# daxiongpro/EPNet

Hardware: AMD Instinct MI355X
Metric: SA-stack points/sec per GPU (16384-pt KITTI scene) + % HBM roofline (higher is better)
Workload: dtype f32

## Files before the change

### epnet_amd/_lib.py

```python
import ctypes
import os

_HERE = os.path.dirname(os.path.abspath(__file__))
LIB_PATH = os.environ.get("EPNET_HIP_LIB") or os.path.join(_HERE, "lib", "libepnet_hip.so")

_vp = ctypes.c_void_p
_i = ctypes.c_int
_f = ctypes.c_float
_sz = ctypes.c_size_t
_i64 = ctypes.c_int64

SIGNATURES = {
    "epnet_abi_version": (_i, []),
    "epnet_strerror": (ctypes.c_char_p, [_i]),
    "epnet_last_hip_error": (ctypes.c_char_p, []),
    "epnet_furthest_point_sampling": (_i, [_i, _i, _i, _vp, _vp, _vp, _vp]),
    "epnet_gather_points": (_i, [_i, _i, _i, _i, _vp, _vp, _vp, _vp]),
    "epnet_gather_points_grad": (_i, [_i, _i, _i, _i, _vp, _vp, _vp, _vp]),
    "epnet_ball_query": (_i, [_i, _i, _i, _f, _i, _vp, _vp, _vp, _vp]),
    "epnet_ball_query_workspace_bytes": (_sz, [_i, _i, _i]),
    "epnet_ball_query_ws": (_i, [_i, _i, _i, _f, _i, _vp, _vp, _vp, _vp, _sz, _vp]),
    "epnet_group_points": (_i, [_i, _i, _i, _i, _i, _vp, _vp, _vp, _vp]),
    "epnet_group_points_grad": (_i, [_i, _i, _i, _i, _i, _vp, _vp, _vp, _vp]),
    "epnet_group_concat": (_i, [_i, _i, _i, _i, _i, _vp, _vp, _vp, _vp, _vp, _i, _vp]),
# ... 5 lines not shown
    "epnet_group_concat_grad_ws": (_i, [_i, _i, _i, _i, _i, _vp, _vp, _vp, _i, _vp, _sz, _vp]),
    "epnet_three_nn": (_i, [_i, _i, _i, _vp, _vp, _vp, _vp, _vp]),
    "epnet_three_nn_workspace_bytes": (_sz, [_i, _i, _i]),
    "epnet_three_nn_ws": (_i, [_i, _i, _i, _vp, _vp, _vp, _vp, _vp, _sz, _vp]),
    "epnet_three_interpolate": (_i, [_i, _i, _i, _i, _vp, _vp, _vp, _vp, _vp]),
    "epnet_three_interpolate_grad": (_i, [_i, _i, _i, _i, _vp, _vp, _vp, _vp, _vp]),
    "epnet_three_interpolate_grad_workspace_bytes": (_sz, [_i, _i, _i]),
    "epnet_three_interpolate_grad_ws": (_i, [_i, _i, _i, _i, _vp, _vp, _vp, _vp, _vp, _sz, _vp]),
    "epnet_group_linear": (_i, [_i, _i, _i, _i, _i, _vp, _vp, _vp, _vp, _vp, _vp, _vp, _vp]),
    "epnet_group_linear_grad_w": (_i, [_i, _i, _i, _i, _i, _vp, _vp, _vp, _vp, _vp, _vp]),
    "epnet_feature_gather": (_i, [_i, _i, _i, _i, _i, _i, _i, _vp, _vp, _vp, _vp, _vp, _vp]),
    "epnet_feature_gather_grad": (_i, [_i, _i, _i, _i, _i, _i, _vp, _vp, _vp, _vp]),
    "epnet_pool_max": (_i, [ctypes.c_longlong, _i, _vp, _vp, _vp, _vp]),
    "epnet_pool_max_grad": (_i, [ctypes.c_longlong, _i, _vp, _vp, _vp, _vp]),
    "epnet_scene_index_bytes": (_sz, [_i, _i]),
    "epnet_scene_index_build": (_i, [_i, _i, _vp, _vp, _sz, _vp]),
    "epnet_scene_index_build_gathered": (_i, [_i, _i, _i, _vp, _vp, _vp, _vp, _sz, _vp]),
    "epnet_furthest_point_sampling_indexed": (_i, [_i, _i, _i, _vp, _vp, _sz, _vp, _vp, _vp]),
    "epnet_sample_centres": (_i, [_i, _i, _i, _vp, _vp, _sz, _vp, _vp, _vp, _vp]),
    "epnet_sample_centres_chain": (_i, [_i, _i, _i, _vp, _vp, _sz, _vp, _vp, _vp, _vp, _vp, _i, _vp]),
    "epnet_group_concat_multi": (_i, [_i, _i, _i, _i, _i, _vp, _vp, _vp, _vp, _vp, _vp, _i, _vp]),
    "epnet_ball_query_indexed_multi": (_i, [_i, _i, _i, _i, _vp, _vp, _vp, _vp, _vp, _sz, _vp, _vp]),
    "epnet_ball_query_ordered": (_i, [_i, _i, _i, _i, _vp, _vp, _vp, _vp, _vp, _sz, _vp, _sz, _vp, _vp]),
    "epnet_three_nn_indexed": (_i, [_i, _i, _i, _vp, _vp, _vp, _sz, _vp, _sz, _vp, _vp, _vp]),
    "epnet_ball_query_indexed": (_i, [_i, _i, _i, _f, _i, _vp, _vp, _vp, _sz, _vp, _vp]),
    "epnet_boxes_overlap_bev": (_i, [_i, _vp, _i, _vp, _vp, _vp]),
    "epnet_boxes_iou_bev": (_i, [_i, _vp, _i, _vp, _vp, _vp]),
    "epnet_boxes_iou3d": (_i, [_i, _vp, _i, _vp, _vp, _vp]),
    "epnet_boxes_iou3d_pairs": (_i, [_i, _vp, _vp, _vp, _vp]),
    "epnet_aug_roi_by_noise": (_i, [_i, _i, _f, _vp, _vp, _vp, _vp, _vp, _vp, _vp, _vp]),
    "epnet_rpn_proposals_workspace_bytes": (_sz, [_i, _i, _i, _i]),
    "epnet_rpn_proposals": (_i, [_i, _i, _vp, _vp, _vp, _i, _i, _i, _f, _i, _vp, _sz, _vp, _vp, _vp, _vp]),
    "epnet_nms_workspace_bytes": (_sz, [_i]),
    "epnet_nms": (_i, [_vp, _i, _f, _vp, _sz, _vp, _vp, _vp]),
    "epnet_nms_normal": (_i, [_vp, _i, _f, _vp, _sz, _vp, _vp, _vp]),
    "epnet_roipool3d_workspace_bytes": (_sz, [_i, _i, _i]),
    "epnet_roipool3d": (_i, [_i, _i, _i, _i, _i, _vp, _vp, _vp, _vp, _vp, _vp, _sz, _vp]),
    "epnet_pts_in_boxes3d_host": (_i, [_vp, _vp, _vp, _i64, _i64]),
    "epnet_roipool3d_host": (_i, [_vp, _vp, _vp, _vp, _vp, _vp, _i64, _i64, _i64, _i64]),
}

_lib = None


class EpnetError(RuntimeError):
    pass
# ... 30 lines not shown
```

### epnet_amd/csrc/ball_query.hip

```cpp
#include <stdlib.h>

#include "common.h"
#include "dpp.h"
#include "spatial.h"

namespace epnet {

constexpr int kBqTile = 2048;
constexpr int kBqThreads = 256;

template <int CPW>
__global__ __launch_bounds__(kBqThreads) void ball_query_kernel(int n, int m, float radius2, int nsample,
                                                                const float *__restrict__ new_xyz,
                                                                const float *__restrict__ xyz,
                                                                int *__restrict__ idx) {
    __shared__ float tile[kBqTile * 3];
    const int lane = threadIdx.x & 63, wave = threadIdx.x >> 6;
    const int bs = blockIdx.y;
    xyz += (size_t)bs * n * 3;
    new_xyz += (size_t)bs * m * 3;
    idx += (size_t)bs * m * nsample;

    const int c0 = (blockIdx.x * (kBqThreads / 64) + wave) * CPW;
    float cx[CPW], cy[CPW], cz[CPW];
// ... 325 lines not shown
        for (int q0 = 0; q0 < nq; q0 += 64) {
            const int qd = q0 + lane;
            const bool qnear = qd < nq && box_near(qboxes + qd * 6, cx, cy, cz, r2);
            const unsigned long long qmask = __ballot(qnear);
            if (!qmask) continue;
            const int nqc = (int)__popcll(qmask);
            if (qnear) quads[popc_below(qmask)] = qd;
            __builtin_amdgcn_wave_barrier();
            for (int s0 = 0; s0 < nqc; s0 += 16) {
                const int slot = s0 + (lane >> 2);
                int bid = 0;
                bool bnear = false;
                if (slot < nqc) {
                    bid = quads[slot] * 4 + (lane & 3);
                    bnear = box_near(boxes + bid * 6, cx, cy, cz, r2);
                }
                scan_buckets(__ballot(bnear), [&](int l) { return __builtin_amdgcn_readlane(bid, l); });
            }
            __builtin_amdgcn_wave_barrier();
        }
    }
}

__device__ __forceinline__ void bq_emit_list(int lane, const int *hits, int cnt, int nsample, int *__restrict__ out) {
    __builtin_amdgcn_wave_barrier();
    const int mine = lane < cnt ? hits[lane] : 0x7fffffff;
    int rank = 0;
    for (int j = 0; j < cnt; ++j) rank += __builtin_amdgcn_readlane(mine, j) < mine ? 1 : 0;
    if (lane < cnt && rank < nsample) out[rank] = mine;
    int first = 0;
    if (cnt) first = __builtin_amdgcn_readlane(mine, (int)__builtin_ctzll(__ballot(lane < cnt && rank == 0)));
    for (int l = cnt + lane; l < nsample; l += 64) out[l] = first;
}

template <int RM>
__device__ __forceinline__ int bq_select_smallest(int lane, int *hits, int cnt, int nsample, int np) {
    __builtin_amdgcn_wave_barrier();
    int key[RM];
#pragma unroll
    for (int r = 0; r < RM; ++r) key[r] = (r * 64 < cnt && r * 64 + lane < cnt) ? hits[r * 64 + lane] : 0x7fffffff;
    int lo = 0, hi = np;
    while (hi - lo > 1) {
        const int mid = (lo + hi) >> 1;
        int c = 0;
#pragma unroll
        for (int r = 0; r < RM; ++r)
            if (r * 64 < cnt) c += (int)__popcll(__ballot(key[r] < mid));
        if (c >= nsample) hi = mid;
        else lo = mid;
    }
    __builtin_amdgcn_wave_barrier();
    int base = 0;
#pragma unroll
    for (int r = 0; r < RM; ++r)
        if (r * 64 < cnt) {
            const bool sel = key[r] < hi;
            const unsigned long long sm = __ballot(sel);
            if (sel) hits[base + popc_below(sm)] = key[r];
            base += (int)__popcll(sm);
        }
    return hi;
}

template <int DPL>
__device__ __forceinline__ void bq_bitmap_search(int lane, int np, float r2, int nsample, float cx, float cy, float cz,
                                                 const float4 *__restrict__ sorted, const float *__restrict__ boxes,
                                                 const float *__restrict__ qboxes, int *__restrict__ out, unsigned *bits,
                                                 int *quads) {
#pragma unroll
    for (int w = 0; w < DPL; ++w) bits[lane * DPL + w] = 0u;
    __builtin_amdgcn_wave_barrier();
    bq_walk<DPL>(lane, np, r2, cx, cy, cz, sorted, boxes, qboxes, quads, [&](const float4 &p, float d2) {
        if (d2 < r2) {
            const int k = __float_as_int(p.w);
            atomicOr(&bits[k >> 5], 1u << (k & 31));
        }
    });
    __builtin_amdgcn_wave_barrier();
    int bc = 0;
#pragma unroll 8
    for (int i = 0; i < DPL; ++i) bc += __popc(bits[lane * DPL + i]);
    const int incl = wave_inclusive_scan(bc);
    const int total = __builtin_amdgcn_readlane(incl, 63);
    int pos = incl - bc;
    int mine_first = 0x7fffffff;
    if (bc > 0 && (pos < nsample || pos == 0)) {
        for (int i = 0; i < DPL; ++i) {
            unsigned ww = bits[lane * DPL + i];
            if (ww && mine_first == 0x7fffffff) mine_first = (lane * DPL + i) * 32 + (int)__builtin_ctz(ww);
            while (ww && pos < nsample) {
                const int bit = (int)__builtin_ctz(ww);
                ww &= ww - 1u;
                out[pos++] = (lane * DPL + i) * 32 + bit;
            }
            if (pos >= nsample) break;
        }
    }
    const unsigned long long have = __ballot(bc > 0);
    int first = 0;
    if (have) first = __builtin_amdgcn_readlane(mine_first, (int)__builtin_ctzll(have));
    for (int l = total + lane; l < nsample; l += 64) out[l] = first;
}

template <int K>
struct BqScales {
    float r2[K];
    int nsample[K];
    int *idx[K];
};

template <int DPL, int K>
__global__ __launch_bounds__(kQThreads) void bq_query_kernel(int np, int m, BqScales<K> sc,
                                                             const float *__restrict__ new_xyz,
                                                             const float4 *__restrict__ sorted,
                                                             const float *__restrict__ boxes,
                                                             const float *__restrict__ qboxes,
                                                             const float4 *__restrict__ order, int npc) {
    __shared__ unsigned s_bits[kQThreads / 64][64 * DPL];
    __shared__ int s_quads[kQThreads / 64][64];
    __shared__ int s_hits[kQThreads / 64][K][64];
    const int lane = threadIdx.x & 63, wave = threadIdx.x >> 6;
    int wg_x, bs;
    xcd_scene_map(wg_x, bs);
    int ci = wg_x * (kQThreads / 64) + wave;
    if (ci >= m) return;
    sorted += (size_t)bs * np;
    boxes += (size_t)bs * (np / 64) * 6;
    qboxes += (size_t)bs * (np / 256) * 6;
    float cx, cy, cz;
    if (order) {
        const float4 e = order[(size_t)bs * npc + ci];
        ci = __float_as_int(e.w);
        cx = e.x; cy = e.y; cz = e.z;
    } else {
        const float *c = new_xyz + ((size_t)bs * m + ci) * 3;
        cx = c[0]; cy = c[1]; cz = c[2];
    }
    float r2max = sc.r2[0];
#pragma unroll
    for (int k = 1; k < K; ++k) r2max = fmaxf(r2max, sc.r2[k]);
    int cnt[K];
#pragma unroll
    for (int k = 0; k < K; ++k) cnt[k] = 0;
    bq_walk<DPL>(lane, np, r2max, cx, cy, cz, sorted, boxes, qboxes, s_quads[wave], [&](const float4 &p, float d2) {
        if (!__ballot(d2 < r2max)) return;
#pragma unroll
        for (int k = 0; k < K; ++k) {
            const bool hit = d2 < sc.r2[k];
            const unsigned long long hm = __ballot(hit);
            if (hm) {
                const int pos = cnt[k] + popc_below(hm);
                if (hit && pos < 64) s_hits[wave][k][pos] = __float_as_int(p.w);
                cnt[k] += (int)__popcll(hm);
            }
        }
    });
#pragma unroll
    for (int k = 0; k < K; ++k) {
        int *out = sc.idx[k] + ((size_t)bs * m + ci) * sc.nsample[k];
        if (cnt[k] <= 64)
            bq_emit_list(lane, s_hits[wave][k], cnt[k], sc.nsample[k], out);
        else
            bq_bitmap_search<DPL>(lane, np, sc.r2[k], sc.nsample[k], cx, cy, cz, sorted, boxes, qboxes, out, s_bits[wave],
                                  s_quads[wave]);
    }
}

template <int DPL, int K, bool kStream>
__global__ __launch_bounds__(kQThreads) void bq_query2_kernel(int np, int m, BqScales<K> sc,
                                                              const float *__restrict__ new_xyz,
                                                              const float4 *__restrict__ sorted,
                                                              const float *__restrict__ boxes,
                                                              const float *__restrict__ qboxes,
                                                              const float4 *__restrict__ order, int npc) {
    constexpr int CAP = kStream ? (K == 1 ? 512 : 256) : 64, kStepAppends = 128;
    constexpr int kBitWords = kStream ? 0 : 64 * DPL;
    __shared__ unsigned s_pool[kQThreads / 64][kBitWords + 2 * K * CAP];
    __shared__ int s_quads[kQThreads / 64][2][64];
    const int lane = threadIdx.x & 63, wave = threadIdx.x >> 6;
    int wg_x, bs;
    xcd_scene_map(wg_x, bs);
    const int ci0 = (wg_x * (kQThreads / 64) + wave) * 2;
    if (ci0 >= m) return;
    const bool two = ci0 + 1 < m;
    sorted += (size_t)bs * np;
    boxes += (size_t)bs * (np / 64) * 6;
    qboxes += (size_t)bs * (np / 256) * 6;
    float ax, ay, az, bx_, by_, bz_;
    int out0 = ci0, out1 = ci0 + 1;
    if (order) {
        const float4 e0 = order[(size_t)bs * npc + ci0], e1 = order[(size_t)bs * npc + ci0 + (two ? 1 : 0)];
        ax = e0.x; ay = e0.y; az = e0.z;
        bx_ = e1.x; by_ = e1.y; bz_ = e1.z;
        out0 = __float_as_int(e0.w);
        out1 = __float_as_int(e1.w);
    } else {
        const float *c0 = new_xyz + ((size_t)bs * m + ci0) * 3;
        const float *c1 = two ? c0 + 3 : c0;
        ax = c0[0]; ay = c0[1]; az = c0[2];
        bx_ = c1[0]; by_ = c1[1]; bz_ = c1[2];
// ... 106 lines not shown
            }
            __builtin_amdgcn_wave_barrier();
        }
    }
#ifdef EPNET_BQ_STATS
    const unsigned long long st_1 = __builtin_amdgcn_s_memtime();
#endif
#pragma unroll
    for (int e = 0; e < 2; ++e) {
        if (e == 1 && !two) break;
        const float cx = e ? bx_ : ax, cy = e ? by_ : ay, cz = e ? bz_ : az;
#pragma unroll
        for (int k = 0; k < K; ++k) {
            int *out = sc.idx[k] + ((size_t)bs * m + (e ? out1 : out0)) * sc.nsample[k];
            int *hits = hits_of + (e * K + k) * CAP;
            if constexpr (kStream) {
                if (cnt[e][k] > 64) {
                    bq_select_smallest<CAP / 64>(lane, hits, cnt[e][k], sc.nsample[k], np);
                    cnt[e][k] = sc.nsample[k];
#ifdef EPNET_BQ_STATS
                    st_sel = true;
#endif
                }
                bq_emit_list(lane, hits, cnt[e][k], sc.nsample[k], out);
            } else {
                if (cnt[e][k] <= 64) {
                    bq_emit_list(lane, hits, cnt[e][k], sc.nsample[k], out);
                } else {
#ifdef EPNET_BQ_STATS
                    st_again = true;
#endif
                    bq_bitmap_search<DPL>(lane, np, sc.r2[k], sc.nsample[k], cx, cy, cz, sorted, boxes, qboxes, out, s_pool[wave],
                                          s_quads[wave][0]);
                }
            }
        }
    }
#ifdef EPNET_BQ_STATS
    {
        const unsigned long long st_3 = __builtin_amdgcn_s_memtime();
        if (lane == 0) {
            const int o = st_again ? 8 : (st_sel ? 4 : 0);
            atomicAdd(&g_bq_stats[o + 0], 1ull);
            atomicAdd(&g_bq_stats[o + 1], st_1 - st_0);
            atomicAdd(&g_bq_stats[o + 2], st_3 - st_1);
            atomicAdd(&g_bq_stats[o + 3], (unsigned long long)st_rows);
            atomicMax(&g_bq_stats[12], st_3 - st_0);
        }
    }
#endif
}

}

using namespace epnet;

extern "C" int epnet_ball_query(int b, int n, int m, float radius, int nsample, const float *new_xyz,
                                const float *xyz, int *idx, epnet_stream_t stream) {
    EPNET_REQUIRE(b >= 0 && n >= 0 && m >= 0 && nsample >= 0);
// ... 12 lines not shown
    }
    return check_launch("ball_query");
}


int epnet::spatial_index_launch(int b, int n, int np, const float *xyz, float4 *sorted, float *boxes, float *qboxes,
                                hipStream_t s, int n_src, const int *src_idx, float *gathered) {
    if (n <= 4096) {
        constexpr int T = 256, cells = 1 << 12;
        const size_t stage = (np & 255) == 0 ? (size_t)(np / 4 < 512 ? np / 4 : 512) * sizeof(float4) : 0;
        hipLaunchKernelGGL((bq_index_kernel<T, 12>), dim3(b), dim3(T), (size_t)(cells + cells / (cells / T) + 64) * sizeof(int) + stage, s,
                           n, np, xyz, sorted, boxes, qboxes, n_src, src_idx, gathered);
    } else {
        constexpr int T = 1024, cells = 1 << 14;
        const size_t stage = (n <= T * 16 && (np & 255) == 0) ? (size_t)(np / 4) * sizeof(float4) : 0;
        hipLaunchKernelGGL((bq_index_kernel<T, 14>), dim3(b), dim3(T), (size_t)(cells + cells / (cells / T) + 64) * sizeof(int) + stage, s,
                           n, np, xyz, sorted, boxes, qboxes, n_src, src_idx, gathered);
    }
    return check_launch("spatial index");
}

template <int K>
static int bq_query_launch(int b, int np, int m, const BqScales<K> &sc, const float *new_xyz, const float4 *sorted,
                           hipStream_t s, const float4 *order = nullptr, int npc = 0) {
    const float *boxes = (const float *)(sorted + (size_t)b * np);
    const float *qboxes = boxes + (size_t)b * (np / 64) * 6;
    const char *pair_str = getenv("EPNET_BQ_PAIR");
    const int pair_env = pair_str ? atoi(pair_str) : -1;
    const bool pair = pair_env >= 0 ? pair_env != 0 : (long long)b * m >= 65536;
    const char *pad_str = getenv("EPNET_BQ_PAD_KB");
    const size_t pad = pad_str ? (size_t)atoi(pad_str) * 1024 : 0;
    if (pair) {
        dim3 grid(div_up(div_up(m, 2), kQThreads / 64), b);
        bool stream = np > 16384;
        if (const char *e = getenv("EPNET_BQ_STREAM")) stream = atoi(e) != 0;
        for (int k = 0; k < K; ++k) stream = stream && sc.nsample[k] <= 64;
#define EPNET_BQ2(D_)                                                                                                                   \
    do {                                                                                                                                \
        if (stream)                                                                                                                     \
            hipLaunchKernelGGL((bq_query2_kernel<D_, K, true>), grid, dim3(kQThreads), pad, s, np, m, sc, new_xyz, sorted, boxes, qboxes, \
                               order, npc);                                                                                             \
        else                                                                                                                            \
            hipLaunchKernelGGL((bq_query2_kernel<D_, K, false>), grid, dim3(kQThreads), pad, s, np, m, sc, new_xyz, sorted, boxes,       \
                               qboxes, order, npc);                                                                                     \
    } while (0)
        switch (np / 2048) {
            case 1: EPNET_BQ2(1); break;
            case 2: EPNET_BQ2(2); break;
            case 4: EPNET_BQ2(4); break;
            case 8: EPNET_BQ2(8); break;
            case 16: EPNET_BQ2(16); break;
            default: EPNET_BQ2(32); break;
        }
#undef EPNET_BQ2
        return check_launch("ball_query query");
    }
    dim3 grid(div_up(m, kQThreads / 64), b);
#define EPNET_BQ(D_) hipLaunchKernelGGL((bq_query_kernel<D_, K>), grid, dim3(kQThreads), pad, s, np, m, sc, new_xyz, sorted, boxes, qboxes, order, npc)
    switch (np / 2048) {
        case 1: EPNET_BQ(1); break;
        case 2: EPNET_BQ(2); break;
        case 4: EPNET_BQ(4); break;
        case 8: EPNET_BQ(8); break;
        case 16: EPNET_BQ(16); break;
        default: EPNET_BQ(32); break;
    }
#undef EPNET_BQ
    return check_launch("ball_query query");
}

extern "C" size_t epnet_scene_index_bytes(int b, int n) { return scene_index_bytes(b, n); }

extern "C" int epnet_scene_index_build(int b, int n, const float *xyz, void *index, size_t index_bytes,
                                       epnet_stream_t stream) {
    const size_t need = scene_index_bytes(b, n);
    EPNET_REQUIRE(need != 0 && xyz && index);
    if (index_bytes < need) return EPNET_ENOMEM;
    if (((uintptr_t)index & 15) != 0) return EPNET_EINVAL;
    EPNET_REQUIRE(b <= 65535);
    const int np = scene_index_np(n);
    float4 *sorted = (float4 *)index;
// ... 35 lines not shown
extern "C" int epnet_ball_query_indexed_multi(int b, int n, int m, int nscales, const float *radii, const int *nsamples,
                                              const float *new_xyz, const float *xyz, const void *index,
                                              size_t index_bytes, int *const *idx, epnet_stream_t stream) {
    EPNET_REQUIRE(nscales >= 0 && (nscales == 0 || (radii && nsamples && idx)));
    const size_t need = scene_index_bytes(b, n);
    bool fused = nscales == 2 && need != 0 && index && m > 0 && nsamples[0] > 0 && nsamples[1] > 0;
    if (!fused) {
        for (int k = 0; k < nscales; ++k) {
            const int rc = epnet_ball_query_indexed(b, n, m, radii[k], nsamples[k], new_xyz, xyz, index, index_bytes, idx[k], stream);
            if (rc) return rc;
        }
        return EPNET_OK;
    }
    EPNET_REQUIRE(new_xyz && idx[0] && idx[1]);
    if (index_bytes < need) return EPNET_ENOMEM;
    EPNET_REQUIRE(b <= 65535);
    BqScales<2> sc;
    for (int k = 0; k < 2; ++k) {
        sc.r2[k] = radii[k] * radii[k];
        sc.nsample[k] = nsamples[k];
        sc.idx[k] = idx[k];
    }
    return bq_query_launch<2>(b, scene_index_np(n), m, sc, new_xyz, (const float4 *)index, (hipStream_t)stream);
}

extern "C" int epnet_ball_query_ordered(int b, int n, int m, int nscales, const float *radii, const int *nsamples,
                                        const float *new_xyz, const float *xyz, const void *index, size_t index_bytes,
                                        const void *centre_index, size_t centre_index_bytes, int *const *idx,
                                        epnet_stream_t stream) {
    EPNET_REQUIRE(nscales >= 0 && (nscales == 0 || (radii && nsamples && idx)));
    const size_t need = scene_index_bytes(b, n), need_c = scene_index_bytes(b, m);
    bool ordered = (nscales == 1 || nscales == 2) && need != 0 && need_c != 0 && index && centre_index && m > 0;
    for (int k = 0; ordered && k < nscales; ++k) ordered = nsamples[k] > 0 && idx[k] != nullptr;
    const char *force = getenv("EPNET_BQ_ORDERED");
    if (force ? atoi(force) == 0 : n <= 16384) ordered = false;
    if (!ordered) return epnet_ball_query_indexed_multi(b, n, m, nscales, radii, nsamples, new_xyz, xyz, index, index_bytes, idx, stream);
    if (index_bytes < need || centre_index_bytes < need_c) return EPNET_ENOMEM;
    EPNET_REQUIRE(b <= 65535);
    const int np = scene_index_np(n), npc = scene_index_np(m);
    if (nscales == 1) {
        BqScales<1> sc;
        sc.r2[0] = radii[0] * radii[0];
        sc.nsample[0] = nsamples[0];
        sc.idx[0] = idx[0];
        return bq_query_launch<1>(b, np, m, sc, new_xyz, (const float4 *)index, (hipStream_t)stream, (const float4 *)centre_index, npc);
    }
// ... 42 lines not shown
```

### epnet_amd/csrc/common.h

```cpp
#pragma once
#include <hip/hip_runtime.h>
#include <stdint.h>

#include "epnet_ops.h"

namespace epnet {

constexpr int kWave = 64;

int record_hip_error(hipError_t e, const char *where);

inline int check_launch(const char *where) {
    hipError_t e = hipGetLastError();
    if (e != hipSuccess) return record_hip_error(e, where);
    return EPNET_OK;
}

inline int div_up(int a, int b) { return (a + b - 1) / b; }
inline long long div_up64(long long a, long long b) { return (a + b - 1) / b; }

__device__ __forceinline__ int lane_id() { return threadIdx.x & (kWave - 1); }

__device__ __forceinline__ int popc_below(unsigned long long mask) {
    return __builtin_amdgcn_mbcnt_hi((unsigned)(mask >> 32), __builtin_amdgcn_mbcnt_lo((unsigned)mask, 0));
}

__device__ __forceinline__ void store_stream(float *dst, float x, float y, float z, float w) {
    typedef float f4 __attribute__((ext_vector_type(4)));
    const f4 v = {x, y, z, w};
    __builtin_nontemporal_store(v, reinterpret_cast<f4 *>(dst));
}

__device__ __forceinline__ void xcd_scene_map(int &wg_x, int &bs) {
// ... 42 lines not shown
```

### epnet_amd/csrc/group.hip

```cpp
#include <stdlib.h>

#include "common.h"
#include "spatial.h"
#include "runsum.h"

namespace epnet {

constexpr int kGThreads = 256;
constexpr int kGChan = 16;

__global__ __launch_bounds__(kGThreads) void gather_rows_vec4_kernel(int c, int n, int p, size_t ostride,
                                                                     const float *__restrict__ points,
                                                                     const int *__restrict__ idx,
                                                                     float *__restrict__ out) {
    int wg_x, wg_y, bs;
    xcd_scene_map3(wg_x, wg_y, bs);
    const int c0 = wg_y * kGChan;
    const int q4 = wg_x * kGThreads + threadIdx.x;
    if (q4 * 4 >= p) return;
    const int4 id = *reinterpret_cast<const int4 *>(idx + (size_t)bs * p + (size_t)q4 * 4);
    const int cend = min(c, c0 + kGChan);
    const float *src = points + ((size_t)bs * c + c0) * n;
    float *dst = out + (size_t)bs * ostride + (size_t)c0 * p + (size_t)q4 * 4;
#pragma unroll 4
// ... 568 lines not shown
    return launch_gather_rows(b, c, n, npoints, points, idx, out, (hipStream_t)stream, "gather_points");
}

extern "C" int epnet_gather_points_grad(int b, int c, int n, int npoints, const float *grad_out, const int *idx,
                                        float *grad_points, epnet_stream_t stream) {
    EPNET_REQUIRE(b >= 0 && c >= 0 && n >= 0 && npoints >= 0);
    return launch_scatter_rows(b, c, n, npoints, grad_out, idx, grad_points, (hipStream_t)stream, "gather_points_grad");
}

extern "C" int epnet_group_points(int b, int c, int n, int npoints, int nsample, const float *points, const int *idx,
                                  float *out, epnet_stream_t stream) {
    EPNET_REQUIRE(b >= 0 && c >= 0 && n >= 0 && npoints >= 0 && nsample >= 0);
    return launch_gather_rows(b, c, n, (long long)npoints * nsample, points, idx, out, (hipStream_t)stream,
                              "group_points");
}

extern "C" int epnet_group_points_grad(int b, int c, int n, int npoints, int nsample, const float *grad_out,
                                       const int *idx, float *grad_points, epnet_stream_t stream) {
    EPNET_REQUIRE(b >= 0 && c >= 0 && n >= 0 && npoints >= 0 && nsample >= 0);
    return launch_scatter_rows(b, c, n, (long long)npoints * nsample, grad_out, idx, grad_points, (hipStream_t)stream,
                               "group_points_grad");
}

static int launch_group_xyz(int b, int n, int npoints, int nsample, long long p, size_t ostride, const float *xyz,
                            const float *new_xyz, const int *idx, float *out, hipStream_t s) {
    if (nsample % 4 == 0 && (((uintptr_t)idx | (uintptr_t)out) % 16 == 0) && (ostride % 4 == 0))
        hipLaunchKernelGGL(group_xyz_centred_vec4_kernel, dim3((unsigned)div_up64(p / 4, kGThreads), b), dim3(kGThreads), 0, s, n,
                           npoints, nsample, ostride, xyz, new_xyz, idx, out);
    else
        hipLaunchKernelGGL(group_xyz_centred_kernel, dim3((unsigned)div_up64(p, kGThreads), b), dim3(kGThreads), 0, s, n, npoints,
                           nsample, ostride, xyz, new_xyz, idx, out);
    return check_launch("group_concat xyz");
}

extern "C" int epnet_group_concat(int b, int c, int n, int npoints, int nsample, const float *xyz, const float *new_xyz,
                                  const float *features, const int *idx, float *out, int use_xyz, epnet_stream_t stream) {
    EPNET_REQUIRE(b >= 0 && c >= 0 && n >= 0 && npoints >= 0 && nsample >= 0);
    EPNET_REQUIRE(use_xyz || c > 0);
    const long long p = (long long)npoints * nsample;
    if (b == 0 || p == 0) return EPNET_OK;
    EPNET_REQUIRE(idx && out && (c == 0 || features) && (!use_xyz || (xyz && new_xyz)));
    EPNET_REQUIRE(n > 0);
    if (p > 0x7fffffffll || b > 65535) return EPNET_ELIMIT;
    hipStream_t s = (hipStream_t)stream;
    const int ch0 = use_xyz ? 3 : 0;
    const size_t ostride = (size_t)(ch0 + c) * (size_t)p;
    if (use_xyz) {
// ... 184 lines not shown
```

### epnet_amd/pointnet2_cuda.py

```python
import torch

from . import _lib
from ._tensor import dev_ptr, need, on_device_of, writes

_F, _I = torch.float32, torch.int32


@writes("idx")
def ball_query_wrapper(b, n, m, radius, nsample, new_xyz, xyz, idx):
    pn, px, pi = dev_ptr(new_xyz, "new_xyz", _F), dev_ptr(xyz, "xyz", _F), dev_ptr(idx, "idx", _I)
    need(new_xyz, b * m * 3, "new_xyz"); need(xyz, b * n * 3, "xyz"); need(idx, b * m * nsample, "idx")
    l = _lib.lib()
    ws_bytes = l.epnet_ball_query_workspace_bytes(b, n, m)
    with on_device_of(xyz) as s:
        if ws_bytes:
            ws = torch.empty((ws_bytes,), dtype=torch.uint8, device=xyz.device)
            _lib.check(l.epnet_ball_query_ws(b, n, m, radius, nsample, pn, px, pi, ws.data_ptr(), ws_bytes, s), "ball_query")
        else:
            _lib.check(l.epnet_ball_query(b, n, m, radius, nsample, pn, px, pi, s), "ball_query")
    return 1


@writes("out")
def group_points_wrapper(b, c, n, npoints, nsample, points, idx, out):
# ... 182 lines not shown
                       "sample_centres")
    return 1


@writes("idxs")
def ball_query_multi_wrapper(b, n, m, radii, nsamples, new_xyz, xyz, index, idxs):
    import ctypes
    pn, pxyz = dev_ptr(new_xyz, "new_xyz", _F), dev_ptr(xyz, "xyz", _F)
    need(new_xyz, b * m * 3, "new_xyz"); need(xyz, b * n * 3, "xyz")
    k = len(radii)
    assert len(nsamples) == k and len(idxs) == k
    ptrs = []
    for ns, t in zip(nsamples, idxs):
        ptrs.append(dev_ptr(t, "idx", _I))
        need(t, b * m * ns, "idx")
    px, nb = _index_args(index, xyz)
    c_r = (ctypes.c_float * k)(*[float(r) for r in radii])
    c_n = (ctypes.c_int * k)(*[int(x) for x in nsamples])
    c_p = (ctypes.c_void_p * k)(*ptrs)
    with on_device_of(xyz) as s:
        _lib.check(_lib.lib().epnet_ball_query_indexed_multi(b, n, m, k, ctypes.cast(c_r, ctypes.c_void_p),
                                                             ctypes.cast(c_n, ctypes.c_void_p), pn, pxyz, px, nb,
                                                             ctypes.cast(c_p, ctypes.c_void_p), s), "ball_query")
    return 1


@writes("idxs")
def ball_query_ordered_wrapper(b, n, m, radii, nsamples, new_xyz, xyz, index, centre_index, idxs):
    import ctypes
    pn, pxyz = dev_ptr(new_xyz, "new_xyz", _F), dev_ptr(xyz, "xyz", _F)
    need(new_xyz, b * m * 3, "new_xyz"); need(xyz, b * n * 3, "xyz")
    k = len(radii)
    assert len(nsamples) == k and len(idxs) == k
    ptrs = []
    for ns, t in zip(nsamples, idxs):
        ptrs.append(dev_ptr(t, "idx", _I))
        need(t, b * m * ns, "idx")
    px, nb = _index_args(index, xyz)
    pc, nc = _index_args(centre_index, new_xyz)
    c_r = (ctypes.c_float * k)(*[float(r) for r in radii])
    c_n = (ctypes.c_int * k)(*[int(x) for x in nsamples])
    c_p = (ctypes.c_void_p * k)(*ptrs)
    with on_device_of(xyz) as s:
        _lib.check(_lib.lib().epnet_ball_query_ordered(b, n, m, k, ctypes.cast(c_r, ctypes.c_void_p), ctypes.cast(c_n, ctypes.c_void_p),
                                                     pn, pxyz, px, nb, pc, nc, ctypes.cast(c_p, ctypes.c_void_p), s), "ball_query")
    return 1
# ... 166 lines not shown
```

### epnet_amd/sa_stack.py

```python
import os

import torch

from . import pointnet2_cuda as ext

RPN_NPOINTS = (4096, 1024, 256, 64)
RPN_RADII = ((0.1, 0.5), (0.5, 1.0), (1.0, 2.0), (2.0, 4.0))
RPN_NSAMPLES = ((16, 32), (16, 32), (16, 32), (16, 32))
RPN_FEAT_CHANNELS = (0, 96, 256, 512)
RPN_FP = ((1024, 64, 256), (512, 256, 1024), (512, 1024, 4096), (256, 4096, 16384))


CONFIGS = {
    2: dict(n=16384, npoints=RPN_NPOINTS, radii=RPN_RADII, nsamples=RPN_NSAMPLES, feat_channels=RPN_FEAT_CHANNELS),
    5: dict(n=65536, npoints=(16384,), radii=((0.5,),), nsamples=((64,),), feat_channels=(64,)),
}


def sa_algorithmic_bytes(n=16384, npoints=RPN_NPOINTS, nsamples=RPN_NSAMPLES, feat_channels=RPN_FEAT_CHANNELS):
    out = {"fps": 0, "gather": 0, "ball_query": 0, "group_xyz": 0, "group_feat": 0}
    cur = n
    for lvl, m in enumerate(npoints):
        out["fps"] += cur * 12 + m * 4
        out["gather"] += m * 4 + 3 * cur * 4 + 3 * m * 4
# ... 40 lines not shown
            chosen = frozenset(int(v) for v in s_query_levels)
        elif queries_in_s is not None:
            chosen = every if queries_in_s else frozenset()
        elif env_lv is not None:
            chosen = frozenset(int(v) for v in env_lv.split(",") if v.strip())
        elif self.stages == 3:
            chosen = every
        elif env_q == 2 or (env_q == 1 and with_fp):
            chosen = every
        elif env_q == 1 and batch * n >= 240 * 16384:
            chosen = every - {0}
        else:
            chosen = frozenset()
        self.s_query_levels = chosen & every
        self.queries_in_s = self.s_query_levels == every
        self.chain = bool(int(os.environ.get("EPNET_SA_CHAIN", "1"))) and fused_sampling
        self.fuse_gather = bool(int(os.environ.get("EPNET_SA_FUSE_GATHER", "1")))
        self._deferred = None
        self.s_first = bool(int(os.environ.get("EPNET_SA_S_FIRST", "0" if self.s_query_levels else "1")))
        self.tail_scales = int(os.environ.get("EPNET_SA_TAIL_SCALES", "0"))
        self.multi_query = bool(int(os.environ.get("EPNET_SA_MULTI_QUERY", "1")))
        self.multi_group = bool(int(os.environ.get("EPNET_SA_MULTI_GROUP", "1")))
        self.ordered_query = bool(int(os.environ.get("EPNET_SA_ORDERED_QUERY", "1")))
        self.side = None
        self.npoints, self.radii, self.nsamples, self.feat_channels = npoints, radii, nsamples, feat_channels
        self.with_fp, self.fp = with_fp, fp
        dev = torch.device(device)
        g = torch.Generator().manual_seed(seed)
        f32, i32 = torch.float32, torch.int32
        self.levels = []
        cur = n
        for lvl, m in enumerate(npoints):
            c = feat_channels[lvl]
            index_bytes = ext.scene_index_bytes(batch, cur) if shared_index else 0
            L = {
                "n": cur, "m": m, "c": c,
                "xyz_t_sets": [torch.empty((batch, 3, cur), dtype=f32, device=dev) for _ in range(self.ring if not fused else 1)],
                "temp": torch.empty((batch, cur), dtype=f32, device=dev),
                "fps_idx_sets": ([torch.empty((batch, m), dtype=i32, device=dev) for _ in range(3)] if self.stages == 3 else None),
                "fps_idx": None,
                "new_xyz_t": torch.empty((batch, 3, m), dtype=f32, device=dev),
                "sets": [{"new_xyz": torch.empty((batch, m, 3), dtype=f32, device=dev),
                          "index": (torch.empty((index_bytes,), dtype=torch.uint8, device=dev) if index_bytes else None),
                          "prefix": torch.zeros((batch,), dtype=i32, device=dev),
                          "centre_index": (torch.empty((ext.scene_index_bytes(batch, m),), dtype=torch.uint8, device=dev)
                                           if (shared_index and lvl + 1 == len(npoints) and ext.scene_index_bytes(batch, m)) else None)}
# ... 140 lines not shown
                                         [self._idx(S, parity) for S in L["scales"]])
        else:
            for S in L["scales"]:
                self._query_scale(L, S, cur_xyz, parity)

    def _centre_index(self, L, parity):
        lvl = self.levels.index(L)
        if lvl + 1 < len(self.levels):
            return self.levels[lvl + 1]["sets"][parity]["index"] if self.shared_index else None
        own = L["sets"][parity].get("centre_index")
        if own is not None:
            ext.scene_index_build_wrapper(self.batch, L["m"], L["sets"][parity]["new_xyz"], own)
        return own

    def _group_scales(self, L, cur_xyz, parity):
        if self.fused and self.multi_group and len(L["scales"]) > 1:
            ext.group_concat_multi_wrapper(self.batch, L["c"], L["n"], L["m"], [S["ns"] for S in L["scales"]], cur_xyz,
                                           L["sets"][parity]["new_xyz"], L["features"], [self._idx(S, parity) for S in L["scales"]],
                                           [S["grouped"] for S in L["scales"]], True)
        else:
            for S in L["scales"]:
                self._group_scale(L, S, cur_xyz, parity)

    def _group_level(self, L, cur_xyz, parity):
        self._query_level(L, cur_xyz, parity)
        self._group_scales(L, cur_xyz, parity)

    def _side_stream(self, device):
        if self.side is None:
            self.side = torch.cuda.Stream(device=device)
        return self.side

    def run(self, xyz):
        main = torch.cuda.current_stream(xyz.device)
        side = self._side_stream(xyz.device) if self.overlap else None
        cur_xyz = xyz
        built = False
        for lvl, L in enumerate(self.levels):
            new_xyz = self._sample_level(L, cur_xyz, 0, index_built=built)
            built = False
            nxt = self.levels[lvl + 1] if lvl + 1 < len(self.levels) else None
            if self.ordered_query and L["n"] > 16384 and nxt is not None and nxt["sets"][0]["index"] is not None:
                ext.scene_index_build_wrapper(self.batch, L["m"], new_xyz, nxt["sets"][0]["index"])
                built = True
            if side is not None:
                side.wait_stream(main)
                with torch.cuda.stream(side):
# ... 209 lines not shown
```

### include/epnet_ops.h

```cpp
#ifndef EPNET_OPS_H
#define EPNET_OPS_H

#include <stddef.h>
#include <stdint.h>

#ifdef __cplusplus
extern "C" {
#endif

#define EPNET_ABI_VERSION 1

#define EPNET_OK 0
#define EPNET_EINVAL (-1)
#define EPNET_ELAUNCH (-2)
#define EPNET_ENOMEM (-3)
#define EPNET_ELIMIT (-4)

typedef void *epnet_stream_t;

int epnet_abi_version(void);
const char *epnet_strerror(int code);
const char *epnet_last_hip_error(void);


// ... 72 lines not shown
                         const float *xy, const int *idx, float *out, float *xy_out, epnet_stream_t stream);
int epnet_feature_gather_grad(int b, int c, int h, int w, int n, int align_corners, const float *grad_out, const float *xy,
                              float *grad_feature_map, epnet_stream_t stream);

size_t epnet_scene_index_bytes(int b, int n);
int epnet_scene_index_build(int b, int n, const float *xyz, void *index, size_t index_bytes, epnet_stream_t stream);
int epnet_scene_index_build_gathered(int b, int n_src, int n, const float *xyz_src, const int *idx, float *gathered, void *index,
                                     size_t index_bytes, epnet_stream_t stream);
int epnet_furthest_point_sampling_indexed(int b, int n, int m, const float *xyz, void *index,
                                          size_t index_bytes, float *temp, int *idx, epnet_stream_t stream);
int epnet_sample_centres(int b, int n, int m, const float *xyz, void *index, size_t index_bytes, float *temp,
                         int *idx, float *new_xyz, epnet_stream_t stream);
int epnet_sample_centres_chain(int b, int n, int m, const float *xyz, void *index, size_t index_bytes, float *temp,
                               int *idx, float *new_xyz, const int *prefix_in, int *prefix_out, int prefix_cap,
                               epnet_stream_t stream);
int epnet_three_nn_indexed(int b, int n, int m, const float *unknown, const float *known, const void *unknown_index,
                           size_t unknown_index_bytes, const void *known_index, size_t known_index_bytes, float *dist2,
                           int *idx, epnet_stream_t stream);
int epnet_ball_query_indexed(int b, int n, int m, float radius, int nsample, const float *new_xyz, const float *xyz,
                             const void *index, size_t index_bytes, int *idx, epnet_stream_t stream);
int epnet_ball_query_indexed_multi(int b, int n, int m, int nscales, const float *radii, const int *nsamples,
                                   const float *new_xyz, const float *xyz, const void *index, size_t index_bytes,
                                   int *const *idx, epnet_stream_t stream);
int epnet_ball_query_ordered(int b, int n, int m, int nscales, const float *radii, const int *nsamples, const float *new_xyz,
                             const float *xyz, const void *index, size_t index_bytes, const void *centre_index,
                             size_t centre_index_bytes, int *const *idx, epnet_stream_t stream);


int epnet_boxes_overlap_bev(int num_a, const float *boxes_a, int num_b, const float *boxes_b,
                            float *ans_overlap, epnet_stream_t stream);

int epnet_boxes_iou_bev(int num_a, const float *boxes_a, int num_b, const float *boxes_b,
                        float *ans_iou, epnet_stream_t stream);

int epnet_boxes_iou3d(int num_a, const float *boxes_a, int num_b, const float *boxes_b, float *ans_iou3d,
                      epnet_stream_t stream);

int epnet_boxes_iou3d_pairs(int k, const float *boxes_a, const float *boxes_b, float *ans_iou3d, epnet_stream_t stream);

int epnet_aug_roi_by_noise(int k, int aug_times, float pos_thresh, float *roi_boxes3d, const float *gt_boxes3d,
                           const float *iou3d_src, const int *tries, const unsigned char *keep_draw,
                           const float *noise, float *iou_of_rois, epnet_stream_t stream);

size_t epnet_rpn_proposals_workspace_bytes(int b, int distance_based, int pre_nms_top_n, int post_nms_top_n);
int epnet_rpn_proposals(int b, int n, const float *proposals, const float *scores, const int64_t *order,
                        int distance_based, int pre_nms_top_n, int post_nms_top_n, float nms_thresh, int rotated,
// ... 32 lines not shown
```

Baseline: 1.340 billion.

## Fuse centred-xyz grouping into ball query kernel for feature-less SA levels

For SA levels with no input features (c==0) that are not on the ordered-query path, the ball query kernel now also writes the centred xyz of each grouped neighbour straight into the grouped output tensor. The neighbour indices are kept in shared memory and reused, so the separate group_xyz launch and its re-read of the idx array go away. The kernels gain an extra template variant and a new C entry point, with a fallback to query-then-group when the shapes or alignment don't fit. Costs are extra shared-memory writes and more register pressure in the query kernels.

```diff
diff --git a/epnet_amd/_lib.py b/epnet_amd/_lib.py
--- a/epnet_amd/_lib.py
+++ b/epnet_amd/_lib.py
@@ -51,6 +51,7 @@
     "epnet_group_concat_multi": (_i, [_i, _i, _i, _i, _i, _vp, _vp, _vp, _vp, _vp, _vp, _i, _vp]),
     "epnet_ball_query_indexed_multi": (_i, [_i, _i, _i, _i, _vp, _vp, _vp, _vp, _vp, _sz, _vp, _vp]),
     "epnet_ball_query_ordered": (_i, [_i, _i, _i, _i, _vp, _vp, _vp, _vp, _vp, _sz, _vp, _sz, _vp, _vp]),
+    "epnet_ball_query_grouped_multi": (_i, [_i, _i, _i, _i, _vp, _vp, _vp, _vp, _vp, _sz, _vp, _vp, _i, _vp]),
     "epnet_three_nn_indexed": (_i, [_i, _i, _i, _vp, _vp, _vp, _sz, _vp, _sz, _vp, _vp, _vp]),
     "epnet_ball_query_indexed": (_i, [_i, _i, _i, _f, _i, _vp, _vp, _vp, _sz, _vp, _vp]),
     "epnet_boxes_overlap_bev": (_i, [_i, _vp, _i, _vp, _vp, _vp]),
diff --git a/epnet_amd/csrc/ball_query.hip b/epnet_amd/csrc/ball_query.hip
--- a/epnet_amd/csrc/ball_query.hip
+++ b/epnet_amd/csrc/ball_query.hip
@@ -371,15 +371,21 @@
     }
 }
 
-__device__ __forceinline__ void bq_emit_list(int lane, const int *hits, int cnt, int nsample, int *__restrict__ out) {
+__device__ __forceinline__ void bq_emit_list(int lane, int *hits, int cnt, int nsample, int *__restrict__ out, bool keep = false) {
     __builtin_amdgcn_wave_barrier();
     const int mine = lane < cnt ? hits[lane] : 0x7fffffff;
     int rank = 0;
     for (int j = 0; j < cnt; ++j) rank += __builtin_amdgcn_readlane(mine, j) < mine ? 1 : 0;
-    if (lane < cnt && rank < nsample) out[rank] = mine;
+    if (lane < cnt && rank < nsample) {
+        out[rank] = mine;
+        if (keep) hits[rank] = mine;
+    }
     int first = 0;
     if (cnt) first = __builtin_amdgcn_readlane(mine, (int)__builtin_ctzll(__ballot(lane < cnt && rank == 0)));
-    for (int l = cnt + lane; l < nsample; l += 64) out[l] = first;
+    for (int l = cnt + lane; l < nsample; l += 64) {
+        out[l] = first;
+        if (keep) hits[l] = first;
+    }
 }
 
 template <int RM>
@@ -415,7 +421,7 @@
 __device__ __forceinline__ void bq_bitmap_search(int lane, int np, float r2, int nsample, float cx, float cy, float cz,
                                                  const float4 *__restrict__ sorted, const float *__restrict__ boxes,
                                                  const float *__restrict__ qboxes, int *__restrict__ out, unsigned *bits,
-                                                 int *quads) {
+                                                 int *quads, int *row = nullptr) {
 #pragma unroll
     for (int w = 0; w < DPL; ++w) bits[lane * DPL + w] = 0u;
     __builtin_amdgcn_wave_barrier();
@@ -440,7 +446,10 @@
             while (ww && pos < nsample) {
                 const int bit = (int)__builtin_ctz(ww);
                 ww &= ww - 1u;
-                out[pos++] = (lane * DPL + i) * 32 + bit;
+                const int k = (lane * DPL + i) * 32 + bit;
+                out[pos] = k;
+                if (row) row[pos] = k;
+                ++pos;
             }
             if (pos >= nsample) break;
         }
@@ -448,7 +457,10 @@
     const unsigned long long have = __ballot(bc > 0);
     int first = 0;
     if (have) first = __builtin_amdgcn_readlane(mine_first, (int)__builtin_ctzll(have));
-    for (int l = total + lane; l < nsample; l += 64) out[l] = first;
+    for (int l = total + lane; l < nsample; l += 64) {
+        out[l] = first;
+        if (row) row[l] = first;
+    }
 }
 
 template <int K>
@@ -456,9 +468,49 @@
     float r2[K];
     int nsample[K];
     int *idx[K];
+    const float *xyz;
+    int n;
+    float *out[K];
+    size_t ostride[K];
 };
 
-template <int DPL, int K>
+template <int E, int K, typename RowOf>
+__device__ __forceinline__ void bq_emit_xyz(int lane, const BqScales<K> &sc, int bs, int m, int ne, const int (&ci)[E],
+                                            const float (&c)[E][3], RowOf &&row_of) {
+    __builtin_amdgcn_wave_barrier();
+    int base = 0, j = -1, ns = 0, cidx = 0;
+    float cx = 0.f, cy = 0.f, cz = 0.f;
+    const int *row = nullptr;
+    float *dst = nullptr;
+    size_t ostride = 0;
+#pragma unroll
+    for (int e = 0; e < E; ++e)
+#pragma unroll
+        for (int k = 0; k < K; ++k) {
+            const int nq = e < ne ? sc.nsample[k] >> 2 : 0;
+            if (lane >= base && lane < base + nq) {
+                j = lane - base;
+                ns = sc.nsample[k];
+                cidx = ci[e];
+                cx = c[e][0]; cy = c[e][1]; cz = c[e][2];
+                row = row_of(e, k);
+                dst = sc.out[k];
+                ostride = sc.ostride[k];
+            }
+            base += nq;
+        }
+    if (j < 0) return;
+    const int4 id = *reinterpret_cast<const int4 *>(row + 4 * j);
+    const float *pts = sc.xyz + (size_t)bs * sc.n * 3;
+    const float *p0 = pts + (size_t)id.x * 3, *p1 = pts + (size_t)id.y * 3, *p2 = pts + (size_t)id.z * 3, *p3 = pts + (size_t)id.w * 3;
+    const size_t p = (size_t)m * ns;
+    float *o = dst + (size_t)bs * ostride + (size_t)cidx * ns + 4 * j;
+    store_stream(o, p0[0] - cx, p1[0] - cx, p2[0] - cx, p3[0] - cx);
+    store_stream(o + p, p0[1] - cy, p1[1] - cy, p2[1] - cy, p3[1] - cy);
+    store_stream(o + 2 * p, p0[2] - cz, p1[2] - cz, p2[2] - cz, p3[2] - cz);
+}
+
+template <int DPL, int K, bool kXyz>
 __global__ __launch_bounds__(kQThreads) void bq_query_kernel(int np, int m, BqScales<K> sc,
                                                              const float *__restrict__ new_xyz,
                                                              const float4 *__restrict__ sorted,
@@ -467,7 +519,7 @@
                                                              const float4 *__restrict__ order, int npc) {
     __shared__ unsigned s_bits[kQThreads / 64][64 * DPL];
     __shared__ int s_quads[kQThreads / 64][64];
-    __shared__ int s_hits[kQThreads / 64][K][64];
+    __shared__ __attribute__((aligned(16))) int s_hits[kQThreads / 64][K][64];
     const int lane = threadIdx.x & 63, wave = threadIdx.x >> 6;
     int wg_x, bs;
     xcd_scene_map(wg_x, bs);
@@ -508,14 +560,19 @@
     for (int k = 0; k < K; ++k) {
         int *out = sc.idx[k] + ((size_t)bs * m + ci) * sc.nsample[k];
         if (cnt[k] <= 64)
-            bq_emit_list(lane, s_hits[wave][k], cnt[k], sc.nsample[k], out);
+            bq_emit_list(lane, s_hits[wave][k], cnt[k], sc.nsample[k], out, kXyz);
         else
             bq_bitmap_search<DPL>(lane, np, sc.r2[k], sc.nsample[k], cx, cy, cz, sorted, boxes, qboxes, out, s_bits[wave],
-                                  s_quads[wave]);
-    }
-}
-
-template <int DPL, int K, bool kStream>
+                                  s_quads[wave], kXyz ? s_hits[wave][k] : nullptr);
+    }
+    if constexpr (kXyz) {
+        const int cis[1] = {ci};
+        const float cs[1][3] = {{cx, cy, cz}};
+        bq_emit_xyz<1, K>(lane, sc, bs, m, 1, cis, cs, [&](int, int k) { return s_hits[wave][k]; });
+    }
+}
+
+template <int DPL, int K, bool kStream, bool kXyz>
 __global__ __launch_bounds__(kQThreads) void bq_query2_kernel(int np, int m, BqScales<K> sc,
                                                               const float *__restrict__ new_xyz,
                                                               const float4 *__restrict__ sorted,
@@ -524,7 +581,7 @@
                                                               const float4 *__restrict__ order, int npc) {
     constexpr int CAP = kStream ? (K == 1 ? 512 : 256) : 64, kStepAppends = 128;
     constexpr int kBitWords = kStream ? 0 : 64 * DPL;
-    __shared__ unsigned s_pool[kQThreads / 64][kBitWords + 2 * K * CAP];
+    __shared__ __attribute__((aligned(16))) unsigned s_pool[kQThreads / 64][kBitWords + 2 * K * CAP];
     __shared__ int s_quads[kQThreads / 64][2][64];
     const int lane = threadIdx.x & 63, wave = threadIdx.x >> 6;
     int wg_x, bs;
@@ -677,19 +734,24 @@
                     st_sel = true;
 #endif
                 }
-                bq_emit_list(lane, hits, cnt[e][k], sc.nsample[k], out);
+                bq_emit_list(lane, hits, cnt[e][k], sc.nsample[k], out, kXyz);
             } else {
                 if (cnt[e][k] <= 64) {
-                    bq_emit_list(lane, hits, cnt[e][k], sc.nsample[k], out);
+                    bq_emit_list(lane, hits, cnt[e][k], sc.nsample[k], out, kXyz);
                 } else {
 #ifdef EPNET_BQ_STATS
                     st_again = true;
 #endif
                     bq_bitmap_search<DPL>(lane, np, sc.r2[k], sc.nsample[k], cx, cy, cz, sorted, boxes, qboxes, out, s_pool[wave],
-                                          s_quads[wave][0]);
+                                          s_quads[wave][0], kXyz ? hits : nullptr);
                 }
             }
         }
+    }
+    if constexpr (kXyz) {
+        const int cis[2] = {out0, out1};
+        const float cs[2][3] = {{ax, ay, az}, {bx_, by_, bz_}};
+        bq_emit_xyz<2, K>(lane, sc, bs, m, two ? 2 : 1, cis, cs, [&](int e, int k) { return hits_of + (e * K + k) * CAP; });
     }
 #ifdef EPNET_BQ_STATS
     {
@@ -748,7 +810,7 @@
 
 template <int K>
 static int bq_query_launch(int b, int np, int m, const BqScales<K> &sc, const float *new_xyz, const float4 *sorted,
-                           hipStream_t s, const float4 *order = nullptr, int npc = 0) {
+                           hipStream_t s, const float4 *order = nullptr, int npc = 0, bool xyz = false) {
     const float *boxes = (const float *)(sorted + (size_t)b * np);
     const float *qboxes = boxes + (size_t)b * (np / 64) * 6;
     const char *pair_str = getenv("EPNET_BQ_PAIR");
@@ -761,14 +823,21 @@
         bool stream = np > 16384;
         if (const char *e = getenv("EPNET_BQ_STREAM")) stream = atoi(e) != 0;
         for (int k = 0; k < K; ++k) stream = stream && sc.nsample[k] <= 64;
-#define EPNET_BQ2(D_)                                                                                                                   \
+#define EPNET_BQ2X(D_, S_)                                                                                                              \
     do {                                                                                                                                \
-        if (stream)                                                                                                                     \
-            hipLaunchKernelGGL((bq_query2_kernel<D_, K, true>), grid, dim3(kQThreads), pad, s, np, m, sc, new_xyz, sorted, boxes, qboxes, \
-                               order, npc);                                                                                             \
+        if (xyz)                                                                                                                        \
+            hipLaunchKernelGGL((bq_query2_kernel<D_, K, S_, true>), grid, dim3(kQThreads), pad, s, np, m, sc, new_xyz, sorted, boxes,    \
+                               qboxes, order, npc);                                                                                     \
         else                                                                                                                            \
-            hipLaunchKernelGGL((bq_query2_kernel<D_, K, false>), grid, dim3(kQThreads), pad, s, np, m, sc, new_xyz, sorted, boxes,       \
+            hipLaunchKernelGGL((bq_query2_kernel<D_, K, S_, false>), grid, dim3(kQThreads), pad, s, np, m, sc, new_xyz, sorted, boxes,   \
                                qboxes, order, npc);                                                                                     \
+    } while (0)
+#define EPNET_BQ2(D_)          \
+    do {                       \
+        if (stream)            \
+            EPNET_BQ2X(D_, true);  \
+        else                   \
+            EPNET_BQ2X(D_, false); \
     } while (0)
         switch (np / 2048) {
             case 1: EPNET_BQ2(1); break;
@@ -779,10 +848,17 @@
             default: EPNET_BQ2(32); break;
         }
 #undef EPNET_BQ2
+#undef EPNET_BQ2X
         return check_launch("ball_query query");
     }
     dim3 grid(div_up(m, kQThreads / 64), b);
-#define EPNET_BQ(D_) hipLaunchKernelGGL((bq_query_kernel<D_, K>), grid, dim3(kQThreads), pad, s, np, m, sc, new_xyz, sorted, boxes, qboxes, order, npc)
+#define EPNET_BQ(D_)                                                                                                                      \
+    do {                                                                                                                                  \
+        if (xyz)                                                                                                                          \
+            hipLaunchKernelGGL((bq_query_kernel<D_, K, true>), grid, dim3(kQThreads), pad, s, np, m, sc, new_xyz, sorted, boxes, qboxes, order, npc);  \
+        else                                                                                                                              \
+            hipLaunchKernelGGL((bq_query_kernel<D_, K, false>), grid, dim3(kQThreads), pad, s, np, m, sc, new_xyz, sorted, boxes, qboxes, order, npc); \
+    } while (0)
     switch (np / 2048) {
         case 1: EPNET_BQ(1); break;
         case 2: EPNET_BQ(2); break;
@@ -864,6 +940,57 @@
         sc.idx[k] = idx[k];
     }
     return bq_query_launch<2>(b, scene_index_np(n), m, sc, new_xyz, (const float4 *)index, (hipStream_t)stream);
+}
+
+extern "C" int epnet_ball_query_grouped_multi(int b, int n, int m, int nscales, const float *radii, const int *nsamples,
+                                              const float *new_xyz, const float *xyz, const void *index, size_t index_bytes,
+                                              int *const *idx, float *const *out, int channels, epnet_stream_t stream) {
+    EPNET_REQUIRE(nscales >= 0 && (nscales == 0 || (radii && nsamples && idx && out)) && channels >= 3);
+    EPNET_REQUIRE(b >= 0 && n >= 0 && m >= 0);
+    if (b == 0 || m == 0) return EPNET_OK;
+    EPNET_REQUIRE(b <= 65535 && new_xyz && xyz);
+    const size_t need = scene_index_bytes(b, n);
+    bool fused = (nscales == 1 || nscales == 2) && need != 0 && index && index_bytes >= need;
+    int lanes = 0;
+    for (int k = 0; k < nscales && fused; ++k) {
+        fused = nsamples[k] > 0 && nsamples[k] <= 64 && nsamples[k] % 4 == 0 && idx[k] && out[k] &&
+                (((uintptr_t)out[k]) % 16 == 0) && (long long)m * nsamples[k] <= 0x7fffffffll;
+        lanes += 2 * (nsamples[k] / 4);
+    }
+    fused = fused && lanes <= 64;
+    if (!fused) {
+        int rc = epnet_ball_query_indexed_multi(b, n, m, nscales, radii, nsamples, new_xyz, xyz, index, index_bytes, idx, stream);
+        for (int k = 0; k < nscales && rc == EPNET_OK; ++k) {
+            const long long p = (long long)m * nsamples[k];
+            if (p > 0) rc = launch_group_xyz(b, n, m, nsamples[k], p, (size_t)channels * (size_t)p, xyz, new_xyz, idx[k], out[k],
+                                             (hipStream_t)stream);
+        }
+        return rc;
+    }
+    const int np = scene_index_np(n);
+    const float4 *sorted = (const float4 *)index;
+    if (nscales == 1) {
+        BqScales<1> sc;
+        sc.r2[0] = radii[0] * radii[0];
+        sc.nsample[0] = nsamples[0];
+        sc.idx[0] = idx[0];
+        sc.xyz = xyz;
+        sc.n = n;
+        sc.out[0] = out[0];
+        sc.ostride[0] = (size_t)channels * (size_t)m * (size_t)nsamples[0];
+        return bq_query_launch<1>(b, np, m, sc, new_xyz, sorted, (hipStream_t)stream, nullptr, 0, true);
+    }
+    BqScales<2> sc;
+    for (int k = 0; k < 2; ++k) {
+        sc.r2[k] = radii[k] * radii[k];
+        sc.nsample[k] = nsamples[k];
+        sc.idx[k] = idx[k];
+        sc.out[k] = out[k];
+        sc.ostride[k] = (size_t)channels * (size_t)m * (size_t)nsamples[k];
+    }
+    sc.xyz = xyz;
+    sc.n = n;
+    return bq_query_launch<2>(b, np, m, sc, new_xyz, sorted, (hipStream_t)stream, nullptr, 0, true);
 }
 
 extern "C" int epnet_ball_query_ordered(int b, int n, int m, int nscales, const float *radii, const int *nsamples,
diff --git a/epnet_amd/csrc/common.h b/epnet_amd/csrc/common.h
--- a/epnet_amd/csrc/common.h
+++ b/epnet_amd/csrc/common.h
@@ -9,6 +9,8 @@
 constexpr int kWave = 64;
 
 int record_hip_error(hipError_t e, const char *where);
+int launch_group_xyz(int b, int n, int npoints, int nsample, long long p, size_t ostride, const float *xyz, const float *new_xyz,
+                     const int *idx, float *out, hipStream_t s);
 
 inline int check_launch(const char *where) {
     hipError_t e = hipGetLastError();
diff --git a/epnet_amd/csrc/group.hip b/epnet_amd/csrc/group.hip
--- a/epnet_amd/csrc/group.hip
+++ b/epnet_amd/csrc/group.hip
@@ -614,7 +614,7 @@
                                "group_points_grad");
 }
 
-static int launch_group_xyz(int b, int n, int npoints, int nsample, long long p, size_t ostride, const float *xyz,
+int epnet::launch_group_xyz(int b, int n, int npoints, int nsample, long long p, size_t ostride, const float *xyz,
                             const float *new_xyz, const int *idx, float *out, hipStream_t s) {
     if (nsample % 4 == 0 && (((uintptr_t)idx | (uintptr_t)out) % 16 == 0) && (ostride % 4 == 0))
         hipLaunchKernelGGL(group_xyz_centred_vec4_kernel, dim3((unsigned)div_up64(p / 4, kGThreads), b), dim3(kGThreads), 0, s, n,
diff --git a/epnet_amd/pointnet2_cuda.py b/epnet_amd/pointnet2_cuda.py
--- a/epnet_amd/pointnet2_cuda.py
+++ b/epnet_amd/pointnet2_cuda.py
@@ -228,6 +228,32 @@
         _lib.check(_lib.lib().epnet_ball_query_indexed_multi(b, n, m, k, ctypes.cast(c_r, ctypes.c_void_p),
                                                              ctypes.cast(c_n, ctypes.c_void_p), pn, pxyz, px, nb,
                                                              ctypes.cast(c_p, ctypes.c_void_p), s), "ball_query")
+    return 1
+
+
+@writes("idxs", "outs")
+def grouped_ball_query_multi_wrapper(b, n, m, radii, nsamples, new_xyz, xyz, index, idxs, outs):
+    import ctypes
+    pn, pxyz = dev_ptr(new_xyz, "new_xyz", _F), dev_ptr(xyz, "xyz", _F)
+    need(new_xyz, b * m * 3, "new_xyz"); need(xyz, b * n * 3, "xyz")
+    k = len(radii)
+    assert len(nsamples) == k and len(idxs) == k and len(outs) == k
+    channels = int(outs[0].shape[1]) if k else 3
+    ptrs, optrs = [], []
+    for ns, t, o in zip(nsamples, idxs, outs):
+        ptrs.append(dev_ptr(t, "idx", _I)); optrs.append(dev_ptr(o, "out", _F))
+        need(t, b * m * ns, "idx")
+        assert o.dim() == 4 and tuple(o.shape) == (b, channels, m, ns), "out: (B, C, m, nsample) with one C for every scale"
+    px, nb = _index_args(index, xyz)
+    c_r = (ctypes.c_float * k)(*[float(r) for r in radii])
+    c_n = (ctypes.c_int * k)(*[int(x) for x in nsamples])
+    c_p = (ctypes.c_void_p * k)(*ptrs)
+    c_o = (ctypes.c_void_p * k)(*optrs)
+    with on_device_of(xyz) as s:
+        _lib.check(_lib.lib().epnet_ball_query_grouped_multi(b, n, m, k, ctypes.cast(c_r, ctypes.c_void_p),
+                                                             ctypes.cast(c_n, ctypes.c_void_p), pn, pxyz, px, nb,
+                                                             ctypes.cast(c_p, ctypes.c_void_p), ctypes.cast(c_o, ctypes.c_void_p),
+                                                             channels, s), "ball_query")
     return 1
 
 
diff --git a/epnet_amd/sa_stack.py b/epnet_amd/sa_stack.py
--- a/epnet_amd/sa_stack.py
+++ b/epnet_amd/sa_stack.py
@@ -86,6 +86,7 @@
         self.multi_query = bool(int(os.environ.get("EPNET_SA_MULTI_QUERY", "1")))
         self.multi_group = bool(int(os.environ.get("EPNET_SA_MULTI_GROUP", "1")))
         self.ordered_query = bool(int(os.environ.get("EPNET_SA_ORDERED_QUERY", "1")))
+        self.query_xyz = bool(int(os.environ.get("EPNET_SA_QUERY_XYZ", "1")))
         self.side = None
         self.npoints, self.radii, self.nsamples, self.feat_channels = npoints, radii, nsamples, feat_channels
         self.with_fp, self.fp = with_fp, fp
@@ -272,7 +273,17 @@
             for S in L["scales"]:
                 self._group_scale(L, S, cur_xyz, parity)
 
+    def _query_groups(self, L, parity):
+        return (self.query_xyz and self.fused and self.multi_query and L["c"] == 0 and L["sets"][parity]["index"] is not None
+                and not (self.ordered_query and L["n"] > 16384))
+
     def _group_level(self, L, cur_xyz, parity):
+        if self._query_groups(L, parity):
+            P = L["sets"][parity]
+            ext.grouped_ball_query_multi_wrapper(self.batch, L["n"], L["m"], [S["radius"] for S in L["scales"]],
+                                                 [S["ns"] for S in L["scales"]], P["new_xyz"], cur_xyz, P["index"],
+                                                 [self._idx(S, parity) for S in L["scales"]], [S["grouped"] for S in L["scales"]])
+            return
         self._query_level(L, cur_xyz, parity)
         self._group_scales(L, cur_xyz, parity)
 
diff --git a/include/epnet_ops.h b/include/epnet_ops.h
--- a/include/epnet_ops.h
+++ b/include/epnet_ops.h
@@ -118,6 +118,9 @@
 int epnet_ball_query_indexed_multi(int b, int n, int m, int nscales, const float *radii, const int *nsamples,
                                    const float *new_xyz, const float *xyz, const void *index, size_t index_bytes,
                                    int *const *idx, epnet_stream_t stream);
+int epnet_ball_query_grouped_multi(int b, int n, int m, int nscales, const float *radii, const int *nsamples,
+                                   const float *new_xyz, const float *xyz, const void *index, size_t index_bytes,
+                                   int *const *idx, float *const *out, int channels, epnet_stream_t stream);
 int epnet_ball_query_ordered(int b, int n, int m, int nscales, const float *radii, const int *nsamples, const float *new_xyz,
                              const float *xyz, const void *index, size_t index_bytes, const void *centre_index,
                              size_t centre_index_bytes, int *const *idx, epnet_stream_t stream);
```

Result: no change. 1.345 billion, median of 6 (+0.4%).
